# Dahan-Wang/Rethinking-Flow-and-Diffusion-Bridge-Models-for-Speech-Enhancement

Hardware: NVIDIA B200
Metric: enhanced audio-sec/sec (5-step SB bridge, ncsnpp_v2) (higher is better)
Workload: dtype fp16

## Files before the change

rethinking-flow-and-diffusion-bridge-models-for-speech-enhancement_b200/csrc/conv_igemm.cu:

```cuda
#include <cuda.h>
#include <mutex>
#include <type_traits>
#include "common.cuh"
#include "tc05.cuh"

namespace fdbm {
int make_act_tile_map(CUtensorMap* map, const op_t* ptr, int B, int T, int F, int C, int box_f, int box_t);
namespace {

using namespace tc05;

constexpr int MT = 2;
constexpr int TILE_T = 16, TILE_F = 8;
constexpr int HALO_T = TILE_T + 2, HALO_F = TILE_F + 2;
constexpr int A_TILE_BYTES = HALO_T * HALO_F * 128;
constexpr int A_TILE_STRIDE = 23552;
#ifndef FDBM_A_STAGES
#define FDBM_A_STAGES 3
#define FDBM_B_STAGES 3
#endif
constexpr int A_STAGES = FDBM_A_STAGES;
constexpr int B_STAGES = FDBM_B_STAGES;
constexpr int BN = 128;
constexpr int B_TILE_BYTES = BN * 128;
// ... 506 lines not shown
              const float* pb = p.pyr_prev + static_cast<int64_t>(tc.b) * Tp * Fp * p.pyr_C;
              if (p.pyr_C == 4) {
                float4 tap[4];
                float wg[4];
#pragma unroll
                for (int u = 0; u < 2; ++u)
#pragma unroll
                  for (int w = 0; w < 2; ++w) {
                    const int tt = t_a + u, ff = f_a + w;
                    const bool ok = tt >= 0 && tt < Tp && ff >= 0 && ff < Fp;
                    wg[u * 2 + w] = ok ? (u ? 1.0f - wt_a : wt_a) * (w ? 1.0f - wf_a : wf_a) : 0.f;
                    tap[u * 2 + w] = ok ? __ldg(reinterpret_cast<const float4*>(pb + (static_cast<int64_t>(tt) * Fp + ff) * 4))
                                        : make_float4(0.f, 0.f, 0.f, 0.f);
                  }
#pragma unroll
                for (int k = 0; k < 4; ++k) {
                  o[0] = fmaf(wg[k], tap[k].x, o[0]); o[1] = fmaf(wg[k], tap[k].y, o[1]);
                  o[2] = fmaf(wg[k], tap[k].z, o[2]); o[3] = fmaf(wg[k], tap[k].w, o[3]);
                }
              } else {
#pragma unroll
                for (int u = 0; u < 2; ++u) {
                  const int tt = t_a + u;
                  if (tt < 0 || tt >= Tp) continue;
                  const float wt = u ? 1.0f - wt_a : wt_a;
#pragma unroll
                  for (int w = 0; w < 2; ++w) {
                    const int ff = f_a + w;
                    if (ff < 0 || ff >= Fp) continue;
                    const float wgt = wt * (w ? 1.0f - wf_a : wf_a);
                    const float* src = pb + (static_cast<int64_t>(tt) * Fp + ff) * p.pyr_C;
                    for (int c = 0; c < p.pyr_C; ++c) o[c] = fmaf(wgt, __ldg(src + c), o[c]);
                  }
                }
              }
            }
            float* dst = p.pyr_out + ((static_cast<int64_t>(tc.b) * p.T + t) * p.F + f) * p.pyr_C;
            if (p.pyr_C == 4) *reinterpret_cast<float4*>(dst) = make_float4(o[0], o[1], o[2], o[3]);
            else for (int c = 0; c < p.pyr_C; ++c) dst[c] = o[c];
          }
          continue;
        }
        const bool full = tc.t0 + TILE_T <= p.T && tc.f0 + TILE_F <= p.F;
        const int64_t tile_base = ((static_cast<int64_t>(tc.b) * p.T + tc.t0) * p.F + tc.f0) * p.Cout + n0 + cc * 4;
        const int roff0 = ((q * 4) * p.F + rsub) * p.Cout, roff_t = p.F * p.Cout, roff_f = 4 * p.Cout;
        auto roff = [&](int it) { return roff0 + (it >> 1) * roff_t + (it & 1) * roff_f; };
        uint32_t okmask = 0;
#pragma unroll
        for (int it = 0; it < 8; ++it) {
          const int m = q * 32 + it * 4 + rsub;
          const bool ok = tc.t0 + (m >> 3) < p.T && tc.f0 + (m & 7) < p.F;
          okmask |= ok ? (1u << it) : 0u;
        }
        const float* res_p = !RES16 && p.residual ? p.residual + tile_base : nullptr;
        const op_t* res16_p = RES16 ? p.residual_h16 + tile_base : nullptr;
        float* of_p = p.out_f32 ? p.out_f32 + tile_base : nullptr;
        op_t* oh_p = p.out_h16 ? p.out_h16 + tile_base : nullptr;
        if (RES16 || res_p) {
          const int nitem = item + gridDim.x;
          const int nct = item_tile(p, nitem);
          const int nmi = nitem < p.n_items ? nct * MT + j : p.n_mtiles;
          const int nblk_n = nitem - nct * p.n_nblocks;
          const TileCoord nt = decode_tile(p, nmi);
          const int t = nt.t0 + (et >> 3), f = nt.f0 + (et & 7);
          if (nt.valid && t < p.T && f < p.F) {
            const int64_t po = ((static_cast<int64_t>(nt.b) * p.T + t) * p.F + f) * p.Cout + nblk_n * BN;
            if (RES16) {
#pragma unroll
              for (int u = 0; u < 2; ++u) asm volatile("prefetch.global.L2 [%0];" ::"l"(p.residual_h16 + po + u * 64));
            } else {
#pragma unroll
              for (int u = 0; u < 4; ++u) asm volatile("prefetch.global.L2 [%0];" ::"l"(p.residual + po + u * 32));
            }
          }
        }
        const float2 sc2 = make_float2(p.scale, p.scale);
        const float* bias_p = p.bias + n0 + cc * 4;
        const float* biasb_p = p.bias_b ? p.bias_b + static_cast<int64_t>(tc.b) * p.bias_b_stride + n0 + cc * 4 : nullptr;
        float4 bv = __ldg(reinterpret_cast<const float4*>(bias_p));
        float4 bvb = biasb_p ? __ldg(reinterpret_cast<const float4*>(biasb_p)) : make_float4(0.f, 0.f, 0.f, 0.f);
        float4 res[8];
#if FDBM_EPI_RES2
        uint2 res16_buf[2][8];
#define res16 res16_buf[ch & 1]
        auto load_res16 = [&](int ch) {
          uint2 (&dst)[8] = res16_buf[ch & 1];
          if (full) {
#pragma unroll
            for (int it = 0; it < 8; ++it) dst[it] = __ldg(reinterpret_cast<const uint2*>(res16_p + roff(it) + ch * 32));
          } else {
#pragma unroll
            for (int it = 0; it < 8; ++it)
              dst[it] = ((okmask >> it) & 1) ? __ldg(reinterpret_cast<const uint2*>(res16_p + roff(it) + ch * 32)) : make_uint2(0u, 0u);
          }
        };
        if (RES16) load_res16(0);
#else
        uint2 res16[8];
        auto load_res16 = [&](int ch) {
          if (full) {
#pragma unroll
            for (int it = 0; it < 8; ++it) res16[it] = __ldg(reinterpret_cast<const uint2*>(res16_p + roff(it) + ch * 32));
          } else {
#pragma unroll
            for (int it = 0; it < 8; ++it)
              res16[it] = ((okmask >> it) & 1) ? __ldg(reinterpret_cast<const uint2*>(res16_p + roff(it) + ch * 32)) : make_uint2(0u, 0u);
          }
        };
#endif
        auto load_res = [&](float4 (&r)[8], int ch) {
          if (full) {
#pragma unroll
            for (int it = 0; it < 8; ++it) r[it] = __ldg(reinterpret_cast<const float4*>(res_p + roff(it) + ch * 32));
          } else {
#pragma unroll
            for (int it = 0; it < 8; ++it)
              r[it] = ((okmask >> it) & 1) ? __ldg(reinterpret_cast<const float4*>(res_p + roff(it) + ch * 32))
                                           : make_float4(0.f, 0.f, 0.f, 0.f);
          }
        };
        const int n_chunks = p.bn >> 5;
#pragma unroll
        for (int ch = 0; ch < BN / 32; ++ch) {
          if (ch >= n_chunks) break;
          float4 cw[4], cbias = make_float4(0.f, 0.f, 0.f, 0.f);
          if constexpr (COMB) {
            const int c = n0 + ch * 32 + cc * 4;
            cbias = __ldg(reinterpret_cast<const float4*>(p.comb_b + c));
#pragma unroll
            for (int u = 0; u < 4; ++u) {
              const float* wr = p.comb_w + (c + u) * p.comb_C;
              cw[u] = make_float4(__ldg(wr), p.comb_C > 1 ? __ldg(wr + 1) : 0.f, p.comb_C > 2 ? __ldg(wr + 2) : 0.f,
                                  p.comb_C > 3 ? __ldg(wr + 3) : 0.f);
            }
          }
          float4 bvn = bv, bvbn = bvb;
          if (ch + 1 < n_chunks) {
            bvn = __ldg(reinterpret_cast<const float4*>(bias_p + (ch + 1) * 32));
            if (biasb_p) bvbn = __ldg(reinterpret_cast<const float4*>(biasb_p + (ch + 1) * 32));
          }
          uint32_t v[32];
          tmem_ld_32x32(tmem_base + ((q * 32u) << 16) + (as * MT + j) * BN + ch * 32, v);
#if FDBM_EPI_RES2
          if (RES16) { if (ch + 1 < n_chunks) load_res16(ch + 1); }
          else if (res_p) load_res(res, ch);
#else
          if (RES16) { if (ch == 0) load_res16(0); }
          else if (res_p) load_res(res, ch);
#endif
          tmem_ld_wait();
#pragma unroll
          for (int g = 0; g < 8; ++g)
            stage[lane * 8 + (g ^ (lane & 7))] = make_float4(__uint_as_float(v[4 * g]), __uint_as_float(v[4 * g + 1]),
                                                             __uint_as_float(v[4 * g + 2]), __uint_as_float(v[4 * g + 3]));
          __syncwarp();
          const float2 bs_lo = __fmul2_rn(make_float2(bv.x + bvb.x, bv.y + bvb.y), sc2), bs_hi = __fmul2_rn(make_float2(bv.z + bvb.z, bv.w + bvb.w), sc2);
          float2 o_lo[8], o_hi[8];
#pragma unroll
          for (int it = 0; it < 8; ++it) {
            const int rr = it * 4 + rsub;
            const float4 a = stage[rr * 8 + (cc ^ (rr & 7))];
            o_lo[it] = make_float2(a.x, a.y); o_hi[it] = make_float2(a.z, a.w);
          }
#pragma unroll
          for (int it = 0; it < 8; ++it) {
            o_lo[it] = __ffma2_rn(o_lo[it], sc2, bs_lo); o_hi[it] = __ffma2_rn(o_hi[it], sc2, bs_hi);
            if (RES16) {
              const op2_t* r2 = reinterpret_cast<const op2_t*>(&res16[it]);
              o_lo[it] = __ffma2_rn(op22f2(r2[0]), sc2, o_lo[it]);
              o_hi[it] = __ffma2_rn(op22f2(r2[1]), sc2, o_hi[it]);
            } else if (res_p) {
              o_lo[it] = __ffma2_rn(make_float2(res[it].x, res[it].y), sc2, o_lo[it]);
              o_hi[it] = __ffma2_rn(make_float2(res[it].z, res[it].w), sc2, o_hi[it]);
            }
            if (COMB && (full || ((okmask >> it) & 1))) {
              const int m = q * 32 + it * 4 + rsub;
              const float* pq = p.comb_pyr + ((static_cast<int64_t>(tc.b) * p.T + tc.t0 + (m >> 3)) * p.F + tc.f0 + (m & 7)) * p.comb_C;
              const float p0 = __ldg(pq), p1 = p.comb_C > 1 ? __ldg(pq + 1) : 0.f, p2 = p.comb_C > 2 ? __ldg(pq + 2) : 0.f,
                          p3 = p.comb_C > 3 ? __ldg(pq + 3) : 0.f;
              o_lo[it].x += cbias.x + cw[0].x * p0 + cw[0].y * p1 + cw[0].z * p2 + cw[0].w * p3;
              o_lo[it].y += cbias.y + cw[1].x * p0 + cw[1].y * p1 + cw[1].z * p2 + cw[1].w * p3;
              o_hi[it].x += cbias.z + cw[2].x * p0 + cw[2].y * p1 + cw[2].z * p2 + cw[2].w * p3;
              o_hi[it].y += cbias.w + cw[3].x * p0 + cw[3].y * p1 + cw[3].z * p2 + cw[3].w * p3;
            }
          }
#if !FDBM_EPI_RES2
          if (RES16 && ch + 1 < n_chunks) load_res16(ch + 1);
#endif
          float2 ssum_lo = make_float2(0.f, 0.f), ssum_hi = ssum_lo, ssq_lo = ssum_lo, ssq_hi = ssum_lo;
          if (full) {
            if (of_p) {
#pragma unroll
              for (int it = 0; it < 8; ++it)
                *reinterpret_cast<float4*>(of_p + roff(it) + ch * 32) = make_float4(o_lo[it].x, o_lo[it].y, o_hi[it].x, o_hi[it].y);
            }
            if (oh_p) {
#pragma unroll
              for (int it = 0; it < 8; ++it)
                *reinterpret_cast<uint2*>(oh_p + roff(it) + ch * 32) = make_uint2(pack_op2(o_lo[it].x, o_lo[it].y), pack_op2(o_hi[it].x, o_hi[it].y));
            }
#pragma unroll
            for (int it = 0; it < 8; ++it) {
              ssum_lo = __fadd2_rn(ssum_lo, o_lo[it]); ssum_hi = __fadd2_rn(ssum_hi, o_hi[it]);
              ssq_lo = __ffma2_rn(o_lo[it], o_lo[it], ssq_lo); ssq_hi = __ffma2_rn(o_hi[it], o_hi[it], ssq_hi);
            }
          } else {
#pragma unroll
            for (int it = 0; it < 8; ++it) {
              if ((okmask >> it) & 1) {
                if (of_p) *reinterpret_cast<float4*>(of_p + roff(it) + ch * 32) = make_float4(o_lo[it].x, o_lo[it].y, o_hi[it].x, o_hi[it].y);
                if (oh_p) *reinterpret_cast<uint2*>(oh_p + roff(it) + ch * 32) = make_uint2(pack_op2(o_lo[it].x, o_lo[it].y), pack_op2(o_hi[it].x, o_hi[it].y));
                ssum_lo = __fadd2_rn(ssum_lo, o_lo[it]); ssum_hi = __fadd2_rn(ssum_hi, o_hi[it]);
                ssq_lo = __ffma2_rn(o_lo[it], o_lo[it], ssq_lo); ssq_hi = __ffma2_rn(o_hi[it], o_hi[it], ssq_hi);
              }
            }
          }
          float4 ssum = make_float4(ssum_lo.x, ssum_lo.y, ssum_hi.x, ssum_hi.y), ssq = make_float4(ssq_lo.x, ssq_lo.y, ssq_hi.x, ssq_hi.y);
          if (do_stats) {
#pragma unroll
            for (int sft = 8; sft <= 16; sft <<= 1) {
              ssum.x += __shfl_xor_sync(0xffffffffu, ssum.x, sft); ssum.y += __shfl_xor_sync(0xffffffffu, ssum.y, sft);
              ssum.z += __shfl_xor_sync(0xffffffffu, ssum.z, sft); ssum.w += __shfl_xor_sync(0xffffffffu, ssum.w, sft);
              ssq.x += __shfl_xor_sync(0xffffffffu, ssq.x, sft); ssq.y += __shfl_xor_sync(0xffffffffu, ssq.y, sft);
              ssq.z += __shfl_xor_sync(0xffffffffu, ssq.z, sft); ssq.w += __shfl_xor_sync(0xffffffffu, ssq.w, sft);
            }
            if (rsub == 0) {
              float4* d = reinterpret_cast<float4*>(wstat + q * BN + ch * 32 + cc * 4);
              d[0] = make_float4(ssum.x, ssq.x, ssum.y, ssq.y);
              d[1] = make_float4(ssum.z, ssq.z, ssum.w, ssq.w);
            }
          }
          __syncwarp();
// ... 153 lines not shown
  PackDesc d{};
  d.w1 = w; d.w2 = nullptr; d.out = wpack; d.kind = 1; d.C1 = Cin; d.ksize = k; d.io = ksize == -1; d.C2 = Cin_total ? Cin_total : Cin; d.Cout = Cout;
  d.rows_total = 0; d.row_offset = ci_off;
  d.total = static_cast<long long>(Cout / 64) * k * k * Cin * 64;
  return d;
}
int launch_pack_batch(const PackDesc* descs_dev, int n_descs, long long n_blocks, cudaStream_t s) {
  if (n_descs <= 0 || n_blocks <= 0) return FDBM_OK;
  pack_batch_kernel<<<static_cast<unsigned>(n_blocks), 256, 0, s>>>(descs_dev, n_descs);
  FDBM_LAUNCH_CHECK();
  return FDBM_OK;
}

__global__ void __launch_bounds__(256) pack_one_kernel(const PackDesc d) {
  for (int64_t i = blockIdx.x * 256ll + threadIdx.x; i < d.total; i += 256ll * gridDim.x) {
    if (d.kind == 0) pack_fwd_element(d, i); else pack_dgrad_element(d, i);
  }
}

int launch_pack_conv_weights(const float* w1, int C1, int ksize, const float* w2, int C2, int Cout, int n_rows_total,
                             int row_offset, op_t* wpack, cudaStream_t s) {
  FDBM_REQUIRE((ksize == -2 && C1 <= 4 && C2 == 0) ||
               (C1 % 64 == 0 && C2 % 64 == 0 && (ksize == 1 || ksize == 3 || ksize == -1)),
               "pack_conv_weights: channels must be multiples of 64, ksize 1 or 3");
  const PackDesc d = pack_desc_fwd(w1, C1, ksize, w2, C2, Cout, n_rows_total, row_offset, wpack);
  pack_one_kernel<<<static_cast<int>(std::min<int64_t>(ceil_div64(d.total, 256), 4096)), 256, 0, s>>>(d);
  FDBM_LAUNCH_CHECK();
  return FDBM_OK;
}

int launch_pack_conv_weights_dgrad(const float* w, int Cout, int Cin, int ksize, op_t* wpack, cudaStream_t s, int Cin_total, int ci_off) {
  FDBM_REQUIRE(Cout % 64 == 0 && Cin % 64 == 0 && (ksize == 1 || ksize == 3 || ksize == -1),
               "pack_conv_weights_dgrad: channels must be multiples of 64, ksize 1, 3 or -1 (NIN)");
  const PackDesc d = pack_desc_dgrad(w, Cout, Cin, ksize, wpack, Cin_total, ci_off);
  pack_one_kernel<<<static_cast<int>(std::min<int64_t>(ceil_div64(d.total, 256), 4096)), 256, 0, s>>>(d);
  FDBM_LAUNCH_CHECK();
  return FDBM_OK;
}

int launch_conv_igemm(const ConvArgs& a, cudaStream_t s) {
  FDBM_REQUIRE(a.n_seg >= 1 && a.n_seg <= MAX_SEG, "conv_igemm: 1..%d K segments", MAX_SEG);
  const int bn = a.narrow_n ? 16 : (a.Cout == 64 ? 64 : BN);
  FDBM_REQUIRE(a.Cout % bn == 0 && (!a.narrow_n || (a.Cout == 16 && a.pyr_out)), "conv_igemm: Cout must be a multiple of %d (got %d)", bn, a.Cout);
  FDBM_REQUIRE(a.out_f32 || a.out_h16 || a.pyr_out, "conv_igemm: no output");
  FDBM_REQUIRE(!a.pyr_out || (a.pyr_C >= 1 && a.pyr_C <= 4 && a.Cout == bn && !a.sums), "conv_igemm: bad pyramid epilogue arguments");
  FDBM_REQUIRE(!a.pyr_prev || (a.T % 2 == 0 && a.F % 2 == 0), "conv_igemm: pyramid level with odd size");
  static PerDeviceOnce attr_once;
  if (attr_once.first(current_device())) {
    FDBM_CUDA(cudaFuncSetAttribute(conv_igemm_kernel<false, false>, cudaFuncAttributeMaxDynamicSharedMemorySize, SMEM_BYTES));
    FDBM_CUDA(cudaFuncSetAttribute(conv_igemm_kernel<false, true>, cudaFuncAttributeMaxDynamicSharedMemorySize, SMEM_BYTES));
    FDBM_CUDA(cudaFuncSetAttribute(conv_igemm_kernel<true, false>, cudaFuncAttributeMaxDynamicSharedMemorySize, SMEM_BYTES));
  }
  FDBM_REQUIRE(!a.comb_pyr || (a.comb_w && a.comb_b && a.comb_C >= 1 && a.comb_C <= 4 && !a.pyr_out), "conv_igemm: bad Combine epilogue arguments");
  CUtensorMap map_a[MAX_SEG], map_b;
  ConvParams p;
  p.B = a.B; p.T = a.T; p.F = a.F; p.Cout = a.Cout;
  p.n_seg = a.n_seg;
  int kb = 0, n_kt = 0;
  for (int i = 0; i < MAX_SEG; ++i) {
    if (i < a.n_seg) {
      const ConvSeg& sg = a.seg[i];
      FDBM_REQUIRE(sg.in && sg.C > 0 && sg.C % 64 == 0 && (sg.taps == 9 || sg.taps == 1),
                   "conv_igemm: segment %d needs a tensor, C %% 64 == 0 and 9 or 1 taps (C=%d, taps=%d)", i, sg.C, sg.taps);
      const int halo = sg.taps == 9 || sg.norm_tab != nullptr;
      if (int rc = halo ? make_act_map(&map_a[i], sg.in, a.B, a.T, a.F, sg.C)
                        : make_act_tile_map(&map_a[i], sg.in, a.B, a.T, a.F, sg.C, TILE_F, TILE_T)) return rc;
      p.seg[i].halo = halo;
      kb += sg.C / 64; p.seg[i].taps = sg.taps;
      p.seg[i].norm = sg.norm_tab != nullptr; p.seg[i].act = sg.act; p.seg[i].tab = sg.norm_tab;
      p.seg[i].tab_stride = sg.tab_stride;
      n_kt += (sg.C / 64) * sg.taps;
    } else {
      map_a[i] = map_a[0];
      p.seg[i] = SegParams{1, 0, 0, 0, 0, nullptr};
    }
  }
  p.n_kb = kb;
  FDBM_REQUIRE(kb <= MAX_KB, "conv_igemm: at most %d K-blocks (got %d)", MAX_KB, kb);
  {
    uint32_t nine[MAX_KB], one[MAX_KB];
    int n9 = 0, n1 = 0, kt = 0;
    for (int i = 0; i < a.n_seg; ++i)
      for (int cb = 0; cb < a.seg[i].C / 64; ++cb) {
        const uint32_t e = static_cast<uint32_t>(i) | (static_cast<uint32_t>(cb) << 4) | (static_cast<uint32_t>(kt) << 16);
        if (a.seg[i].taps == 9) nine[n9++] = e; else one[n1++] = e;
        kt += a.seg[i].taps;
      }
    static const int order = getenv("FDBM_KSCHED") ? atoi(getenv("FDBM_KSCHED")) : 0;
    int n = 0;
    if (order == 1) {
      for (int i = 0; i < n1; ++i) p.ksched[n++] = one[i];
      for (int i = 0; i < n9; ++i) p.ksched[n++] = nine[i];
    } else if (order == 2 && n9 > 0) {
      p.ksched[n++] = nine[0];
      for (int i = 0; i < n1; ++i) p.ksched[n++] = one[i];
      for (int i = 1; i < n9; ++i) p.ksched[n++] = nine[i];
    } else {
      for (int i = 0; i < n9; ++i) p.ksched[n++] = nine[i];
      for (int i = 0; i < n1; ++i) p.ksched[n++] = one[i];
    }
    for (; n < MAX_KB; ++n) p.ksched[n] = 0;
    bool side_ok = order == 0 && n1 > 0 && n9 > 0;
    for (int i = 0; i < a.n_seg; ++i) side_ok = side_ok && (a.seg[i].taps == 9 || !p.seg[i].halo);
    static const int side_env = getenv("FDBM_SIDE_RING") ? atoi(getenv("FDBM_SIDE_RING")) : FDBM_SIDE_RING_DEFAULT;
    p.side_ring = side_ok && side_env ? 1 : 0;
    p.n_main = p.side_ring ? n9 : kb;
    p.side_gap = p.side_ring ? std::max(3, ceil_div(9 * n9, n1)) : 0;
    p.n_steps = n_kt;
  }
  if (int rc = make_weight_map(&map_b, a.wpack, static_cast<int64_t>(n_kt) * a.Cout, bn)) return rc;
  p.bn = bn;
  p.tiles_t = ceil_div(a.T, TILE_T); p.tiles_f = ceil_div(a.F, TILE_F);
  p.n_mtiles = a.B * p.tiles_t * p.tiles_f;
  p.n_nblocks = a.Cout / bn;
  p.n_items = ceil_div(p.n_mtiles, MT) * p.n_nblocks;
  {
    auto magic = [](int d) { return static_cast<uint32_t>((0x100000000ull + d - 1) / static_cast<uint64_t>(d)); };
    p.mg_tiles_t = magic(p.tiles_t); p.mg_tiles_f = magic(p.tiles_f); p.mg_nblocks = magic(p.n_nblocks);
    const int64_t dmax = std::max(std::max(p.tiles_t, p.tiles_f), p.n_nblocks);
    FDBM_REQUIRE((2 * (static_cast<int64_t>(p.n_items) + num_sms()) + 2) * dmax < 0x100000000ll, "conv_igemm: %d items exceed the range of the index arithmetic", p.n_items);
  }
  p.bias = a.bias; p.bias_b = a.bias_b; p.bias_b_stride = a.bias_b_stride; p.residual = a.residual; p.scale = a.scale;
  p.residual_h16 = a.residual_h16;
  FDBM_REQUIRE(!(a.residual && a.residual_h16) && !(a.residual_h16 && (a.comb_pyr || a.pyr_out)), "conv_igemm: bad residual arguments");
  p.out_f32 = a.out_f32; p.out_h16 = a.out_h16; p.sums = a.sums;
  p.pyr_out = a.pyr_out; p.pyr_prev = a.pyr_prev; p.pyr_C = a.pyr_C;
  p.comb_pyr = a.comb_pyr; p.comb_w = a.comb_w; p.comb_b = a.comb_b; p.comb_C = a.comb_C;
  if (a.sums) {
    FDBM_REQUIRE(p.n_nblocks <= STAT_SLOTS, "conv_igemm: channel sums support Cout <= %d", STAT_SLOTS * BN);
    if (!a.sums_prezeroed) FDBM_CUDA(cudaMemsetAsync(a.sums, 0, sizeof(double) * 2 * a.B * a.Cout, s));
  }
  const int grid = std::min(p.n_items, num_sms());
  cudaLaunchConfig_t cfg = {};
  cfg.gridDim = dim3(grid); cfg.blockDim = dim3(NUM_THREADS); cfg.dynamicSmemBytes = SMEM_BYTES; cfg.stream = s;
  cudaLaunchAttribute attr[1];
  attr[0].id = cudaLaunchAttributeProgrammaticStreamSerialization;
  attr[0].val.programmaticStreamSerializationAllowed = 1;
  cfg.attrs = attr; cfg.numAttrs = pdl_enabled() && a.B <= pdl_batch_limit() ? 1 : 0;
  if (a.comb_pyr) FDBM_CUDA(cudaLaunchKernelEx(&cfg, conv_igemm_kernel<true, false>, map_a[0], map_a[1], map_a[2], map_b, p));
  else if (a.residual_h16) FDBM_CUDA(cudaLaunchKernelEx(&cfg, conv_igemm_kernel<false, true>, map_a[0], map_a[1], map_a[2], map_b, p));
  else FDBM_CUDA(cudaLaunchKernelEx(&cfg, conv_igemm_kernel<false, false>, map_a[0], map_a[1], map_a[2], map_b, p));
  FDBM_LAUNCH_CHECK();
  return FDBM_OK;
}

}

using namespace fdbm;

extern "C" int fdbm_pack_conv_weights(const float* w1, int C1, int ksize, const float* w2, int C2, int Cout,
                                      void* wpack, int64_t* bytes, void* stream) {
  const int k = ksize == -1 ? 1 : ksize;
  if (bytes) *bytes = ksize == -2 ? static_cast<int64_t>(Cout) * 64 * 2 : conv_wpack_bytes(C1, k, C2, Cout);
  if (!wpack) return FDBM_OK;
  if (int rc = require_sm100()) return rc;
  FDBM_REQUIRE(w1 && ((C2 == 0) == (w2 == nullptr)), "fdbm_pack_conv_weights: null pointer");
  FDBM_REQUIRE(ksize != -2 || (C1 >= 1 && 9 * C1 <= 64 && C2 == 0), "fdbm_pack_conv_weights: ksize -2 needs 9 * C1 <= 64 and no second operand");
  return launch_pack_conv_weights(w1, C1, ksize, w2, C2, Cout, Cout, 0, reinterpret_cast<op_t*>(wpack),
                                  as_stream(stream));
}

extern "C" int fdbm_pack_conv_weights_dgrad(const float* w, int Cout, int Cin, int ksize, void* wpack, int64_t* bytes,
                                            void* stream) {
  const int k = ksize == -1 ? 1 : ksize;
  if (bytes) *bytes = conv_wpack_bytes(Cout, k, 0, Cin);
  if (!wpack) return FDBM_OK;
  if (int rc = require_sm100()) return rc;
  FDBM_REQUIRE(w, "fdbm_pack_conv_weights_dgrad: null weights");
  return launch_pack_conv_weights_dgrad(w, Cout, Cin, ksize, reinterpret_cast<op_t*>(wpack), as_stream(stream));
}

extern "C" int fdbm_conv_igemm(const void* in1, int C1, int ksize, const void* in2, int C2, const void* wpack,
                               const float* bias, const float* bias_b, const float* residual, float scale, int batch,
                               int T, int F, int Cout, float* out_f32, void* out_h16, double* sums, void* stream) {
  if (int rc = require_sm100()) return rc;
  FDBM_REQUIRE(in1 && wpack && bias && batch > 0 && T > 0 && F > 0, "fdbm_conv_igemm: bad arguments");
  FDBM_REQUIRE(ksize == 1 || ksize == 3, "fdbm_conv_igemm: ksize must be 1 or 3");
// ... 34 lines not shown
```

rethinking-flow-and-diffusion-bridge-models-for-speech-enhancement_b200/csrc/norm_resample.cu:

```cuda
#include "common.cuh"

namespace fdbm {
namespace {

struct Taps1D {
  int n;
  int pos[4];
  float w[4];
};

__device__ __forceinline__ Taps1D taps_for(int o, int mode) {
  Taps1D t;
  if (mode == 1) {
    t.n = 4;
    t.pos[0] = 2 * o - 1; t.pos[1] = 2 * o; t.pos[2] = 2 * o + 1; t.pos[3] = 2 * o + 2;
    t.w[0] = 0.125f; t.w[1] = 0.375f; t.w[2] = 0.375f; t.w[3] = 0.125f;
  } else if (mode == 2) {
    const int i = o >> 1;
    t.n = 2;
    if (o & 1) { t.pos[0] = i; t.pos[1] = i + 1; t.w[0] = 0.75f; t.w[1] = 0.25f; }
    else       { t.pos[0] = i - 1; t.pos[1] = i; t.w[0] = 0.25f; t.w[1] = 0.75f; }
    t.pos[2] = t.pos[3] = -1; t.w[2] = t.w[3] = 0.f;
  } else {
    t.n = 1; t.pos[0] = o; t.w[0] = 1.f;
    t.pos[1] = t.pos[2] = t.pos[3] = -1; t.w[1] = t.w[2] = t.w[3] = 0.f;
  }
  return t;
}

__host__ __device__ inline int out_dim(int n, int mode) { return mode == 1 ? n / 2 : (mode == 2 ? n * 2 : n); }

__global__ void __launch_bounds__(256)
fir_resample_kernel(const float* __restrict__ in, int B, int T, int F, int C, int mode, float scale, float* __restrict__ out) {
  const int To = out_dim(T, mode), Fo = out_dim(F, mode);
  const int64_t total = static_cast<int64_t>(B) * To * Fo * C;
  for (int64_t i = blockIdx.x * 256ll + threadIdx.x; i < total; i += 256ll * gridDim.x) {
    const int c = static_cast<int>(i % C);
    int64_t p = i / C;
    const int fo = static_cast<int>(p % Fo); p /= Fo;
    const int to = static_cast<int>(p % To);
    const int b = static_cast<int>(p / To);
    const Taps1D tt = taps_for(to, mode), tf = taps_for(fo, mode);
    float acc = 0.f;
    for (int a = 0; a < tt.n; ++a) {
      if (tt.pos[a] < 0 || tt.pos[a] >= T) continue;
      for (int q = 0; q < tf.n; ++q) {
        if (tf.pos[q] < 0 || tf.pos[q] >= F) continue;
        acc += tt.w[a] * tf.w[q] * in[((static_cast<int64_t>(b) * T + tt.pos[a]) * F + tf.pos[q]) * C + c];
      }
    }
    out[i] = acc * scale;
  }
}

__global__ void __launch_bounds__(256)
channel_stats_kernel(const float* __restrict__ in, int64_t P, int C, int64_t px_per_block, double* __restrict__ sums) {
  __shared__ float4 red_s[256], red_q[256];
  const int cg = C / 4;
  const int pl = 256 / cg;
  const int ci = threadIdx.x % cg, pi = threadIdx.x / cg;
  const int b = blockIdx.y;
  const int64_t p0 = blockIdx.x * px_per_block;
  const int64_t p1 = min(P, p0 + px_per_block);
  float4 s = make_float4(0.f, 0.f, 0.f, 0.f), q = s;
  if (pi < pl) {
    const float4* base = reinterpret_cast<const float4*>(in + static_cast<int64_t>(b) * P * C) + ci;
    for (int64_t p = p0 + pi; p < p1; p += pl) {
      const float4 v = base[p * cg];
      s.x += v.x; s.y += v.y; s.z += v.z; s.w += v.w;
      q.x += v.x * v.x; q.y += v.y * v.y; q.z += v.z * v.z; q.w += v.w * v.w;
    }
  }
  red_s[threadIdx.x] = s;
  red_q[threadIdx.x] = q;
  __syncthreads();
  if (threadIdx.x < cg) {
    double ds[4] = {0, 0, 0, 0}, dq[4] = {0, 0, 0, 0};
    for (int j = 0; j < pl; ++j) {
      const float4 a = red_s[j * cg + threadIdx.x], c2 = red_q[j * cg + threadIdx.x];
      ds[0] += a.x; ds[1] += a.y; ds[2] += a.z; ds[3] += a.w;
      dq[0] += c2.x; dq[1] += c2.y; dq[2] += c2.z; dq[3] += c2.w;
    }
    double* o = sums + (static_cast<int64_t>(b) * C + threadIdx.x * 4) * 2;
#pragma unroll
    for (int j = 0; j < 4; ++j) {
      atomicAdd(o + 2 * j, ds[j]);
      atomicAdd(o + 2 * j + 1, dq[j]);
    }
  }
}

constexpr int GN_MAXC = 512;


template <int MODE, bool SRC16>
__global__ void __launch_bounds__(256)
groupnorm_act_kernel(const void* __restrict__ src1, const double* __restrict__ sums1, int C1,
                     const void* __restrict__ src2, const double* __restrict__ sums2, int C2,
                     const float* __restrict__ gamma, const float* __restrict__ beta, int T, int F, int silu,
                     int px_per_block, uint4* __restrict__ act_out, uint4* __restrict__ raw_out) {
  pdl_wait_then_trigger();
  __shared__ float sA[GN_MAXC], sB[GN_MAXC];
  __shared__ float s_mean[32], s_rstd[32];
  const int C = C1 + C2;
  const int b = blockIdx.y;
// ... 41 lines not shown

  const int To = out_dim(T, MODE), Fo = out_dim(F, MODE);
  const int n_px = To * Fo;
  const int p0 = blockIdx.x * px_per_block;
  const int p1 = min(n_px, p0 + px_per_block);
  constexpr int NT = MODE == 1 ? 4 : (MODE == 2 ? 2 : 1);
  for (int p = p0 + pl; p < p1; p += npl) {
    const int fo = p % Fo, to = p / Fo;
    float acc[8], raw[8];
#pragma unroll
    for (int j = 0; j < 8; ++j) { acc[j] = 0.f; raw[j] = 0.f; }
    const Taps1D tt = taps_for(to, MODE), tf = taps_for(fo, MODE);
#pragma unroll
    for (int u = 0; u < NT; ++u) {
      if (tt.pos[u] < 0 || tt.pos[u] >= T) continue;
#pragma unroll
      for (int v = 0; v < NT; ++v) {
        if (tf.pos[v] < 0 || tf.pos[v] >= F) continue;
        const float w = tt.w[u] * tf.w[v];
        const int64_t off = (static_cast<int64_t>(tt.pos[u]) * F + tf.pos[v]) * Cs + cs;
        float x[8];
        if (SRC16) {
          const uint4 rawv = *reinterpret_cast<const uint4*>(sh + off);
          const op2_t* h2 = reinterpret_cast<const op2_t*>(&rawv);
#pragma unroll
          for (int j = 0; j < 4; ++j) { const float2 f2 = op22f2(h2[j]); x[2 * j] = f2.x; x[2 * j + 1] = f2.y; }
        } else {
          const float4 x0 = *reinterpret_cast<const float4*>(sf + off), x1 = *reinterpret_cast<const float4*>(sf + off + 4);
          x[0] = x0.x; x[1] = x0.y; x[2] = x0.z; x[3] = x0.w; x[4] = x1.x; x[5] = x1.y; x[6] = x1.z; x[7] = x1.w;
        }
#pragma unroll
        for (int j = 0; j < 8; ++j) {
          float y = fmaf(x[j], a[j], bb[j]);
          if (silu) {
            float th;
            asm("tanh.approx.f32 %0, %1;" : "=f"(th) : "f"(0.5f * y));
            y *= fmaf(th, 0.5f, 0.5f);
          }
          acc[j] = fmaf(w, y, acc[j]);
          raw[j] = fmaf(w, x[j], raw[j]);
        }
      }
    }
    const int64_t o = (static_cast<int64_t>(b) * n_px + p) * cg8 + g8;
    act_out[o] = make_uint4(pack_op2(acc[0], acc[1]), pack_op2(acc[2], acc[3]), pack_op2(acc[4], acc[5]),
                            pack_op2(acc[6], acc[7]));
    if (raw_out)
      raw_out[o] = make_uint4(pack_op2(raw[0], raw[1]), pack_op2(raw[2], raw[3]), pack_op2(raw[4], raw[5]),
                              pack_op2(raw[6], raw[7]));
  }
}

constexpr int RS_ROWS = 16;

template <int MODE>
__global__ void __launch_bounds__(256, 2)
gn_resample16_kernel(const op_t* __restrict__ src1, int C1, const op_t* __restrict__ src2, int C2,
                     const float2* __restrict__ tab, int B, int T, int F, op_t* __restrict__ act_out,
                     op_t* __restrict__ raw_out) {
  const int C = C1 + C2, C4 = C / 4;
  const int To = MODE == 1 ? T / 2 : T * 2, Fo = MODE == 1 ? F / 2 : F * 2;
  const int nstrip = MODE == 1 ? (Fo + 1) / 2 : (F + 1) / 2;
  const int nrows = MODE == 1 ? To : T;
  const int nchunk = (nrows + RS_ROWS - 1) / RS_ROWS;
  int64_t idx = blockIdx.x * 256ll + threadIdx.x;
  if (idx >= static_cast<int64_t>(B) * nchunk * nstrip * C4) return;
  const int cg = static_cast<int>(idx % C4); idx /= C4;
  const int strip = static_cast<int>(idx % nstrip); idx /= nstrip;
  const int chunk = static_cast<int>(idx % nchunk);
  const int b = static_cast<int>(idx / nchunk);
  const int c0 = cg * 4;
  const bool from2 = c0 >= C1;
  const int Cs = from2 ? C2 : C1;
  const op_t* sp = (from2 ? src2 : src1) + static_cast<int64_t>(b) * T * F * Cs + (from2 ? c0 - C1 : c0);
  float2 sc[2], sh[2];
  {
    const float4* tp = reinterpret_cast<const float4*>(tab + static_cast<int64_t>(b) * C + c0);
    const float4 e0 = __ldg(tp), e1 = __ldg(tp + 1);
    sc[0] = make_float2(0.5f * e0.x, 0.5f * e0.z); sh[0] = make_float2(0.5f * e0.y, 0.5f * e0.w);
    sc[1] = make_float2(0.5f * e1.x, 0.5f * e1.z); sh[1] = make_float2(0.5f * e1.y, 0.5f * e1.w);
  }
  auto px_act = [&](const uint2 rawv, float2 (&a)[2], float2 (&r)[2]) {
    const op2_t* h2 = reinterpret_cast<const op2_t*>(&rawv);
#pragma unroll
    for (int w = 0; w < 2; ++w) {
      r[w] = op22f2(h2[w]);
      const float2 y = __ffma2_rn(r[w], sc[w], sh[w]);
      const op2_t h = f2op2(y.x, y.y);
      a[w] = op22f2(__hfma2(h, op2_tanh(h), h));
    }
  };
  auto store_px = [&](int to, int fo, const float2 (&a)[2], const float2 (&r)[2]) {
    if (fo >= Fo) return;
    const int64_t o = ((static_cast<int64_t>(b) * To + to) * Fo + fo) * C + c0;
    *reinterpret_cast<uint2*>(act_out + o) = make_uint2(pack_op2(a[0].x, a[0].y), pack_op2(a[1].x, a[1].y));
    *reinterpret_cast<uint2*>(raw_out + o) = make_uint2(pack_op2(r[0].x, r[0].y), pack_op2(r[1].x, r[1].y));
  };
  const float2 zero2 = make_float2(0.f, 0.f);

  if (MODE == 1) {
    const int fo0 = 2 * strip, fi0 = 2 * fo0 - 1;
    uint32_t okf = 0;
#pragma unroll
    for (int k = 0; k < 6; ++k) okf |= (fi0 + k >= 0 && fi0 + k < F) ? (1u << k) : 0u;
    const float2 w1 = make_float2(0.125f, 0.125f), w3 = make_float2(0.375f, 0.375f);
    auto load_row = [&](int t, uint2 (&raw)[6]) {
      const bool in = t >= 0 && t < T;
      const op_t* rp = sp + (static_cast<int64_t>(in ? t : 0) * F + fi0) * Cs;
#pragma unroll
      for (int k = 0; k < 6; ++k) raw[k] = (in && ((okf >> k) & 1)) ? __ldg(reinterpret_cast<const uint2*>(rp + k * Cs)) : make_uint2(0u, 0u);
    };
    auto hrow = [&](int t, const uint2 (&raw)[6], float2 (&ha)[2][2], float2 (&hr)[2][2]) {
#pragma unroll
      for (int j = 0; j < 2; ++j) { ha[j][0] = zero2; ha[j][1] = zero2; hr[j][0] = zero2; hr[j][1] = zero2; }
      if (t < 0 || t >= T) return;
#pragma unroll
      for (int k = 0; k < 6; ++k) {
        float2 a[2], r[2];
        px_act(raw[k], a, r);
        if (!((okf >> k) & 1)) { a[0] = zero2; a[1] = zero2; }
        if (k < 4) {
          const float2 w = (k == 0 || k == 3) ? w1 : w3;
#pragma unroll
          for (int c = 0; c < 2; ++c) { ha[0][c] = __ffma2_rn(w, a[c], ha[0][c]); hr[0][c] = __ffma2_rn(w, r[c], hr[0][c]); }
        }
        if (k >= 2) {
          const float2 w = (k == 2 || k == 5) ? w1 : w3;
#pragma unroll
          for (int c = 0; c < 2; ++c) { ha[1][c] = __ffma2_rn(w, a[c], ha[1][c]); hr[1][c] = __ffma2_rn(w, r[c], hr[1][c]); }
        }
      }
    };
    const int to0 = chunk * RS_ROWS, to1 = min(To, to0 + RS_ROWS);
    float2 ca[2][2], cr[2][2], na[2][2], nr[2][2], ha[2][2], hr[2][2];
    uint2 ra[6], rb[6], qa[6], qb[6];
    load_row(2 * to0 - 1, ra); load_row(2 * to0, rb);
    load_row(2 * to0 + 1, qa); load_row(2 * to0 + 2, qb);
    hrow(2 * to0 - 1, ra, ha, hr);
#pragma unroll
    for (int j = 0; j < 2; ++j)
#pragma unroll
      for (int c = 0; c < 2; ++c) { ca[j][c] = __fmul2_rn(w1, ha[j][c]); cr[j][c] = __fmul2_rn(w1, hr[j][c]); }
    hrow(2 * to0, rb, ha, hr);
#pragma unroll
    for (int j = 0; j < 2; ++j)
#pragma unroll
      for (int c = 0; c < 2; ++c) { ca[j][c] = __ffma2_rn(w3, ha[j][c], ca[j][c]); cr[j][c] = __ffma2_rn(w3, hr[j][c], cr[j][c]); }
#pragma unroll 1
    for (int to = to0; to < to1; ++to) {
#pragma unroll
      for (int k = 0; k < 6; ++k) { ra[k] = qa[k]; rb[k] = qb[k]; }
      if (to + 1 < to1) { load_row(2 * to + 3, qa); load_row(2 * to + 4, qb); }
      hrow(2 * to + 1, ra, ha, hr);
#pragma unroll
      for (int j = 0; j < 2; ++j)
#pragma unroll
        for (int c = 0; c < 2; ++c) {
          ca[j][c] = __ffma2_rn(w3, ha[j][c], ca[j][c]); cr[j][c] = __ffma2_rn(w3, hr[j][c], cr[j][c]);
          na[j][c] = __fmul2_rn(w1, ha[j][c]); nr[j][c] = __fmul2_rn(w1, hr[j][c]);
        }
      hrow(2 * to + 2, rb, ha, hr);
#pragma unroll
      for (int j = 0; j < 2; ++j) {
#pragma unroll
        for (int c = 0; c < 2; ++c) {
          ca[j][c] = __ffma2_rn(w1, ha[j][c], ca[j][c]); cr[j][c] = __ffma2_rn(w1, hr[j][c], cr[j][c]);
          na[j][c] = __ffma2_rn(w3, ha[j][c], na[j][c]); nr[j][c] = __ffma2_rn(w3, hr[j][c], nr[j][c]);
        }
        store_px(to, fo0 + j, ca[j], cr[j]);
#pragma unroll
        for (int c = 0; c < 2; ++c) { ca[j][c] = na[j][c]; cr[j][c] = nr[j][c]; }
      }
    }
  } else {
    const int f0 = 2 * strip;
    uint32_t okf = 0;
#pragma unroll
    for (int k = 0; k < 4; ++k) okf |= (f0 - 1 + k >= 0 && f0 - 1 + k < F) ? (1u << k) : 0u;
    const float2 q1 = make_float2(0.25f, 0.25f), q3 = make_float2(0.75f, 0.75f);
    auto hrow = [&](int t, float2 (&ha)[4][2], float2 (&hr)[4][2]) {
      float2 a[4][2], r[4][2];
      if (t < 0 || t >= T) {
#pragma unroll
        for (int k = 0; k < 4; ++k) { ha[k][0] = zero2; ha[k][1] = zero2; hr[k][0] = zero2; hr[k][1] = zero2; }
        return;
      }
      const op_t* rp = sp + (static_cast<int64_t>(t) * F + f0 - 1) * Cs;
      uint2 raw[4];
#pragma unroll
      for (int k = 0; k < 4; ++k) raw[k] = ((okf >> k) & 1) ? __ldg(reinterpret_cast<const uint2*>(rp + k * Cs)) : make_uint2(0u, 0u);
#pragma unroll
      for (int k = 0; k < 4; ++k) {
        px_act(raw[k], a[k], r[k]);
        if (!((okf >> k) & 1)) { a[k][0] = zero2; a[k][1] = zero2; }
      }
#pragma unroll
      for (int c = 0; c < 2; ++c) {
        ha[0][c] = __ffma2_rn(q1, a[0][c], __fmul2_rn(q3, a[1][c])); hr[0][c] = __ffma2_rn(q1, r[0][c], __fmul2_rn(q3, r[1][c]));
        ha[1][c] = __ffma2_rn(q3, a[1][c], __fmul2_rn(q1, a[2][c])); hr[1][c] = __ffma2_rn(q3, r[1][c], __fmul2_rn(q1, r[2][c]));
        ha[2][c] = __ffma2_rn(q1, a[1][c], __fmul2_rn(q3, a[2][c])); hr[2][c] = __ffma2_rn(q1, r[1][c], __fmul2_rn(q3, r[2][c]));
        ha[3][c] = __ffma2_rn(q3, a[2][c], __fmul2_rn(q1, a[3][c])); hr[3][c] = __ffma2_rn(q3, r[2][c], __fmul2_rn(q1, r[3][c]));
      }
    };
    const int i0 = chunk * RS_ROWS, i1 = min(T, i0 + RS_ROWS);
    float2 pa[4][2], pr[4][2], qa[4][2], qr[4][2];
    hrow(i0 - 1, pa, pr);
#pragma unroll 1
    for (int i = i0; i <= i1; ++i) {
      hrow(i, qa, qr);
#pragma unroll
      for (int k = 0; k < 4; ++k) {
        float2 oa[2], orr[2];
        if (i > i0) {
#pragma unroll
// ... 44 lines not shown
    }
    const double cnt = cpg * pixels;
    const double mean = s / cnt;
    double var = q / cnt - mean * mean;
    if (var < 0) var = 0;
    s_mean[threadIdx.x] = static_cast<float>(mean);
    s_rstd[threadIdx.x] = static_cast<float>(1.0 / sqrt(var + 1e-6));
    if (stats) stats[static_cast<int64_t>(b) * G + threadIdx.x] = make_float2(s_mean[threadIdx.x], s_rstd[threadIdx.x]);
  }
  __syncthreads();
#pragma unroll
  for (int u = 0; u < GN_MAXC / 256; ++u) {
    const int c = threadIdx.x + u * 256;
    if (c < C) {
      if (blk_real && (c & 127) >= blk_real) { table[static_cast<int64_t>(b) * C + c] = make_float2(0.f, 0.f); continue; }
      const int g = (blk_real ? (c >> 7) * blk_real + (c & 127) : c) / cpg;
      const float a = gam[u] * s_rstd[g];
      table[static_cast<int64_t>(b) * C + c] = make_float2(a, bet[u] - s_mean[g] * a);
    }
  }
}

}

int launch_gn_finalize(const double* sums1, int C1, const double* sums2, int C2, const float* gamma, const float* beta,
                       int B, int64_t pixels, float2* table, cudaStream_t s, int blk_real, float2* stats) {
  const int C = C1 + C2;
  FDBM_REQUIRE(blk_real == 0 || (blk_real > 0 && blk_real < 128 && blk_real % 4 == 0 && C1 % 128 == 0 && C2 % 128 == 0),
               "gn_finalize: channel_block_real %d needs 128-channel blocks (%d+%d)", blk_real, C1, C2);
  const int Cr = blk_real ? C / 128 * blk_real : C;
  FDBM_REQUIRE(Cr % std::min(Cr / 4, 32) == 0 && C >= 4 && C <= GN_MAXC, "gn_finalize: unsupported channels %d+%d", C1, C2);
  cudaLaunchConfig_t cfg = {};
  cfg.gridDim = dim3(B); cfg.blockDim = dim3(256); cfg.stream = s;
  cudaLaunchAttribute attr[1];
  attr[0].id = cudaLaunchAttributeProgrammaticStreamSerialization;
  attr[0].val.programmaticStreamSerializationAllowed = 1;
  cfg.attrs = attr; cfg.numAttrs = pdl_enabled() && B <= pdl_batch_limit() ? 1 : 0;
  FDBM_CUDA(cudaLaunchKernelEx(&cfg, gn_finalize_kernel, sums1, C1, sums2, C2, gamma, beta, static_cast<double>(pixels), table, blk_real, stats));
  FDBM_LAUNCH_CHECK();
  return FDBM_OK;
}

int launch_gn_resample16(const op_t* src1, int C1, const op_t* src2, int C2, const float2* tab, int B, int T, int F,
                         int mode, op_t* act_out, op_t* raw_out, cudaStream_t s) {
  const int C = C1 + C2;
  FDBM_REQUIRE(src1 && tab && act_out && raw_out && C1 % 4 == 0 && C2 % 4 == 0 && (C2 == 0) == (src2 == nullptr),
               "gn_resample16: bad arguments (channels %d+%d)", C1, C2);
  FDBM_REQUIRE(mode == 1 || mode == 2, "gn_resample16: mode must be 1 (down) or 2 (up)");
  FDBM_REQUIRE(mode != 1 || (T % 2 == 0 && F % 2 == 0), "gn_resample16: down-sampling needs even T, F");
  const int nstrip = mode == 1 ? (F / 2 + 1) / 2 : (F + 1) / 2;
  const int nrows = mode == 1 ? T / 2 : T;
  const int64_t total = static_cast<int64_t>(B) * ceil_div(nrows, RS_ROWS) * nstrip * (C / 4);
  const unsigned grid = static_cast<unsigned>(ceil_div64(total, 256));
  if (mode == 1) gn_resample16_kernel<1><<<grid, 256, 0, s>>>(src1, C1, src2, C2, tab, B, T, F, act_out, raw_out);
  else gn_resample16_kernel<2><<<grid, 256, 0, s>>>(src1, C1, src2, C2, tab, B, T, F, act_out, raw_out);
  FDBM_LAUNCH_CHECK();
  return FDBM_OK;
}

int launch_fir_resample(const float* in, int B, int T, int F, int C, int mode, float* out, cudaStream_t s) {
  return launch_fir_resample_scaled(in, B, T, F, C, mode, 1.0f, out, s);
}

int launch_fir_resample_scaled(const float* in, int B, int T, int F, int C, int mode, float scale, float* out, cudaStream_t s) {
  const int64_t total = static_cast<int64_t>(B) * out_dim(T, mode) * out_dim(F, mode) * C;
  const int grid = static_cast<int>(std::min<int64_t>(ceil_div64(total, 256), static_cast<int64_t>(num_sms()) * 16));
  fir_resample_kernel<<<grid, 256, 0, s>>>(in, B, T, F, C, mode, scale, out);
  FDBM_LAUNCH_CHECK();
  return FDBM_OK;
}

int launch_channel_stats(const float* in, int B, int T, int F, int C, double* sums, cudaStream_t s) {
  FDBM_REQUIRE(C % 4 == 0 && C / 4 <= 256 && 256 % (C / 4) == 0, "channel_stats: unsupported channel count %d", C);
  FDBM_CUDA(cudaMemsetAsync(sums, 0, sizeof(double) * 2 * B * C, s));
  const int64_t P = static_cast<int64_t>(T) * F;
  const int pl = 256 / (C / 4);
  int64_t blocks_x = std::max<int64_t>(1, (static_cast<int64_t>(num_sms()) * 8) / B);
  blocks_x = std::min<int64_t>(blocks_x, std::max<int64_t>(1, P / (pl * 8)));
  const int64_t ppb = ceil_div64(P, blocks_x);
  dim3 grid(static_cast<unsigned>(ceil_div64(P, ppb)), B);
  channel_stats_kernel<<<grid, 256, 0, s>>>(in, P, C, ppb, sums);
  FDBM_LAUNCH_CHECK();
  return FDBM_OK;
}

int launch_groupnorm_act(const void* src1, int src1_h16, const double* sums1, int C1, const void* src2,
                         const double* sums2, int C2, const float* gamma, const float* beta, int B, int T, int F,
                         int silu, int mode, op_t* act_out, op_t* raw_out, cudaStream_t s) {
  const int C = C1 + C2;
  FDBM_REQUIRE(C <= GN_MAXC && C1 % 8 == 0 && C2 % 8 == 0 && C % std::min(C / 4, 32) == 0 && C / 8 <= 256,
               "groupnorm_act: unsupported channels %d+%d", C1, C2);
  FDBM_REQUIRE(mode >= 0 && mode <= 2, "groupnorm_act: bad mode %d", mode);
  FDBM_REQUIRE(mode != 1 || (T % 2 == 0 && F % 2 == 0), "groupnorm_act: down-sampling needs even T, F");
  const int n_px = out_dim(T, mode) * out_dim(F, mode);
  const int npl = 256 / (C / 8);
  int blocks_x = std::max(1, (num_sms() * 8) / B);
  blocks_x = std::min(blocks_x, std::max(1, n_px / (npl * 4)));
  const int ppb = ceil_div(ceil_div(n_px, blocks_x), npl) * npl;
  dim3 grid(ceil_div(n_px, ppb), B);
  uint4* ao = reinterpret_cast<uint4*>(act_out);
  uint4* ro = reinterpret_cast<uint4*>(raw_out);
#define FDBM_GN_LAUNCH(M, H) \
  FDBM_CUDA(launch_maybe_pdl(groupnorm_act_kernel<M, H>, grid, dim3(256), 0, s, pdl_enabled() && B <= pdl_batch_limit(), src1, sums1, C1, src2, sums2, C2, \
                             gamma, beta, T, F, silu, ppb, ao, ro))
  if (src1_h16) {
    if (mode == 0) FDBM_GN_LAUNCH(0, true); else if (mode == 1) FDBM_GN_LAUNCH(1, true); else FDBM_GN_LAUNCH(2, true);
  } else {
    if (mode == 0) FDBM_GN_LAUNCH(0, false); else if (mode == 1) FDBM_GN_LAUNCH(1, false); else FDBM_GN_LAUNCH(2, false);
  }
#undef FDBM_GN_LAUNCH
  FDBM_LAUNCH_CHECK();
  return FDBM_OK;
}

}

using namespace fdbm;

// ... 38 lines not shown
```

Measured before the change: 1354.

## Hoist Combine pyramid loads, vectorize FIR resample, cp.async ring in down-resample

The Combine epilogue now loads each pixel's pyramid values once per tile, as float4 when four channels are present, instead of reloading them per channel chunk. It also prefetches the next tile's pyramid data and reads the combine weights as float4. A float4 FIR resample kernel replaces the scalar one when alignment and sizes allow. The down-sampling GN resample kernel now streams input rows through a multi-stage cp.async shared-memory ring instead of register double-buffering, which costs dynamic shared memory and could reduce occupancy.

```diff
diff --git a/rethinking-flow-and-diffusion-bridge-models-for-speech-enhancement_b200/csrc/conv_igemm.cu b/rethinking-flow-and-diffusion-bridge-models-for-speech-enhancement_b200/csrc/conv_igemm.cu
--- a/rethinking-flow-and-diffusion-bridge-models-for-speech-enhancement_b200/csrc/conv_igemm.cu
+++ b/rethinking-flow-and-diffusion-bridge-models-for-speech-enhancement_b200/csrc/conv_igemm.cu
@@ -582,7 +582,7 @@
           const bool ok = tc.t0 + (m >> 3) < p.T && tc.f0 + (m & 7) < p.F;
           okmask |= ok ? (1u << it) : 0u;
         }
-        const float* res_p = !RES16 && p.residual ? p.residual + tile_base : nullptr;
+        const float* res_p = !RES16 && !COMB && p.residual ? p.residual + tile_base : nullptr;
         const op_t* res16_p = RES16 ? p.residual_h16 + tile_base : nullptr;
         float* of_p = p.out_f32 ? p.out_f32 + tile_base : nullptr;
         op_t* oh_p = p.out_h16 ? p.out_h16 + tile_base : nullptr;
@@ -649,6 +649,23 @@
                                            : make_float4(0.f, 0.f, 0.f, 0.f);
           }
         };
+        float4 pyr[8];
+        if constexpr (COMB) {
+          const float* pq = p.comb_pyr + ((static_cast<int64_t>(tc.b) * p.T + tc.t0) * p.F + tc.f0) * p.comb_C;
+#pragma unroll
+          for (int it = 0; it < 8; ++it) {
+            const int m = q * 32 + it * 4 + rsub;
+            const float* px = pq + ((m >> 3) * p.F + (m & 7)) * p.comb_C;
+            if (!full && !((okmask >> it) & 1)) pyr[it] = make_float4(0.f, 0.f, 0.f, 0.f);
+            else if (p.comb_C == 4) pyr[it] = __ldg(reinterpret_cast<const float4*>(px));
+            else pyr[it] = make_float4(__ldg(px), p.comb_C > 1 ? __ldg(px + 1) : 0.f, p.comb_C > 2 ? __ldg(px + 2) : 0.f, 0.f);
+          }
+          const int nitem = item + gridDim.x;
+          const TileCoord nt = decode_tile(p, nitem < p.n_items ? item_tile(p, nitem) * MT + j : p.n_mtiles);
+          const int t = nt.t0 + (et >> 3), f = nt.f0 + (et & 7);
+          if (nt.valid && t < p.T && f < p.F)
+            asm volatile("prefetch.global.L2 [%0];" ::"l"(p.comb_pyr + ((static_cast<int64_t>(nt.b) * p.T + t) * p.F + f) * p.comb_C));
+        }
         const int n_chunks = p.bn >> 5;
 #pragma unroll
         for (int ch = 0; ch < BN / 32; ++ch) {
@@ -660,8 +677,8 @@
 #pragma unroll
             for (int u = 0; u < 4; ++u) {
               const float* wr = p.comb_w + (c + u) * p.comb_C;
-              cw[u] = make_float4(__ldg(wr), p.comb_C > 1 ? __ldg(wr + 1) : 0.f, p.comb_C > 2 ? __ldg(wr + 2) : 0.f,
-                                  p.comb_C > 3 ? __ldg(wr + 3) : 0.f);
+              cw[u] = p.comb_C == 4 ? __ldg(reinterpret_cast<const float4*>(wr))
+                                    : make_float4(__ldg(wr), p.comb_C > 1 ? __ldg(wr + 1) : 0.f, p.comb_C > 2 ? __ldg(wr + 2) : 0.f, 0.f);
             }
           }
           float4 bvn = bv, bvbn = bvb;
@@ -704,10 +721,7 @@
               o_hi[it] = __ffma2_rn(make_float2(res[it].z, res[it].w), sc2, o_hi[it]);
             }
             if (COMB && (full || ((okmask >> it) & 1))) {
-              const int m = q * 32 + it * 4 + rsub;
-              const float* pq = p.comb_pyr + ((static_cast<int64_t>(tc.b) * p.T + tc.t0 + (m >> 3)) * p.F + tc.f0 + (m & 7)) * p.comb_C;
-              const float p0 = __ldg(pq), p1 = p.comb_C > 1 ? __ldg(pq + 1) : 0.f, p2 = p.comb_C > 2 ? __ldg(pq + 2) : 0.f,
-                          p3 = p.comb_C > 3 ? __ldg(pq + 3) : 0.f;
+              const float p0 = pyr[it].x, p1 = pyr[it].y, p2 = pyr[it].z, p3 = pyr[it].w;
               o_lo[it].x += cbias.x + cw[0].x * p0 + cw[0].y * p1 + cw[0].z * p2 + cw[0].w * p3;
               o_lo[it].y += cbias.y + cw[1].x * p0 + cw[1].y * p1 + cw[1].z * p2 + cw[1].w * p3;
               o_hi[it].x += cbias.z + cw[2].x * p0 + cw[2].y * p1 + cw[2].z * p2 + cw[2].w * p3;
@@ -967,6 +981,8 @@
     FDBM_CUDA(cudaFuncSetAttribute(conv_igemm_kernel<true, false>, cudaFuncAttributeMaxDynamicSharedMemorySize, SMEM_BYTES));
   }
   FDBM_REQUIRE(!a.comb_pyr || (a.comb_w && a.comb_b && a.comb_C >= 1 && a.comb_C <= 4 && !a.pyr_out), "conv_igemm: bad Combine epilogue arguments");
+  FDBM_REQUIRE(!a.comb_pyr || a.comb_C != 4 || ((reinterpret_cast<uintptr_t>(a.comb_pyr) | reinterpret_cast<uintptr_t>(a.comb_w)) & 15) == 0,
+               "conv_igemm: the 4-channel Combine pyramid and weights must be 16-byte aligned");
   CUtensorMap map_a[MAX_SEG], map_b;
   ConvParams p;
   p.B = a.B; p.T = a.T; p.F = a.F; p.Cout = a.Cout;
@@ -1037,7 +1053,7 @@
   }
   p.bias = a.bias; p.bias_b = a.bias_b; p.bias_b_stride = a.bias_b_stride; p.residual = a.residual; p.scale = a.scale;
   p.residual_h16 = a.residual_h16;
-  FDBM_REQUIRE(!(a.residual && a.residual_h16) && !(a.residual_h16 && (a.comb_pyr || a.pyr_out)), "conv_igemm: bad residual arguments");
+  FDBM_REQUIRE(!(a.residual && a.residual_h16) && !((a.residual || a.residual_h16) && (a.comb_pyr || a.pyr_out)), "conv_igemm: bad residual arguments");
   p.out_f32 = a.out_f32; p.out_h16 = a.out_h16; p.sums = a.sums;
   p.pyr_out = a.pyr_out; p.pyr_prev = a.pyr_prev; p.pyr_C = a.pyr_C;
   p.comb_pyr = a.comb_pyr; p.comb_w = a.comb_w; p.comb_b = a.comb_b; p.comb_C = a.comb_C;
diff --git a/rethinking-flow-and-diffusion-bridge-models-for-speech-enhancement_b200/csrc/norm_resample.cu b/rethinking-flow-and-diffusion-bridge-models-for-speech-enhancement_b200/csrc/norm_resample.cu
--- a/rethinking-flow-and-diffusion-bridge-models-for-speech-enhancement_b200/csrc/norm_resample.cu
+++ b/rethinking-flow-and-diffusion-bridge-models-for-speech-enhancement_b200/csrc/norm_resample.cu
@@ -51,6 +51,31 @@
     }
     out[i] = acc * scale;
   }
+}
+
+__global__ void __launch_bounds__(256)
+fir_resample4_kernel(const float4* __restrict__ in, int T, int F, int C4, int mode, float scale, float4* __restrict__ out) {
+  const int To = out_dim(T, mode), Fo = out_dim(F, mode);
+  const int i = blockIdx.x * 256 + threadIdx.x;
+  if (i >= To * Fo * C4) return;
+  const int b = blockIdx.y;
+  const int c = i % C4, px = i / C4;
+  const int fo = px % Fo, to = px / Fo;
+  const float4* src = in + static_cast<int64_t>(b) * T * F * C4 + c;
+  const Taps1D tt = taps_for(to, mode), tf = taps_for(fo, mode);
+  float4 acc = make_float4(0.f, 0.f, 0.f, 0.f);
+#pragma unroll
+  for (int a = 0; a < 4; ++a) {
+    if (a >= tt.n || tt.pos[a] < 0 || tt.pos[a] >= T) continue;
+#pragma unroll
+    for (int q = 0; q < 4; ++q) {
+      if (q >= tf.n || tf.pos[q] < 0 || tf.pos[q] >= F) continue;
+      const float w = tt.w[a] * tf.w[q];
+      const float4 x = __ldg(src + (tt.pos[a] * F + tf.pos[q]) * C4);
+      acc.x += w * x.x; acc.y += w * x.y; acc.z += w * x.z; acc.w += w * x.w;
+    }
+  }
+  out[static_cast<int64_t>(b) * To * Fo * C4 + i] = make_float4(acc.x * scale, acc.y * scale, acc.z * scale, acc.w * scale);
 }
 
 __global__ void __launch_bounds__(256)
@@ -198,12 +223,25 @@
 }
 
 constexpr int RS_ROWS = 16;
+#ifndef FDBM_RS_STAGES
+#define FDBM_RS_STAGES 3
+#endif
+constexpr int RS_STAGES = FDBM_RS_STAGES;
+constexpr int RS_RING_BYTES = RS_STAGES * 12 * 256 * 8;
+
+__device__ __forceinline__ void cp_async8(void* dst, const void* src, bool ok) {
+  asm volatile("cp.async.ca.shared.global [%0], [%1], 8, %2;" ::"r"(static_cast<uint32_t>(__cvta_generic_to_shared(dst))), "l"(src), "r"(ok ? 8 : 0) : "memory");
+}
+__device__ __forceinline__ void cp_async_commit() { asm volatile("cp.async.commit_group;" ::: "memory"); }
+template <int N>
+__device__ __forceinline__ void cp_async_wait() { asm volatile("cp.async.wait_group %0;" ::"n"(N) : "memory"); }
 
 template <int MODE>
 __global__ void __launch_bounds__(256, 2)
 gn_resample16_kernel(const op_t* __restrict__ src1, int C1, const op_t* __restrict__ src2, int C2,
                      const float2* __restrict__ tab, int B, int T, int F, op_t* __restrict__ act_out,
                      op_t* __restrict__ raw_out) {
+  extern __shared__ uint2 rs_ring[];
   const int C = C1 + C2, C4 = C / 4;
   const int To = MODE == 1 ? T / 2 : T * 2, Fo = MODE == 1 ? F / 2 : F * 2;
   const int nstrip = MODE == 1 ? (Fo + 1) / 2 : (F + 1) / 2;
@@ -250,11 +288,32 @@
 #pragma unroll
     for (int k = 0; k < 6; ++k) okf |= (fi0 + k >= 0 && fi0 + k < F) ? (1u << k) : 0u;
     const float2 w1 = make_float2(0.125f, 0.125f), w3 = make_float2(0.375f, 0.375f);
-    auto load_row = [&](int t, uint2 (&raw)[6]) {
-      const bool in = t >= 0 && t < T;
-      const op_t* rp = sp + (static_cast<int64_t>(in ? t : 0) * F + fi0) * Cs;
-#pragma unroll
-      for (int k = 0; k < 6; ++k) raw[k] = (in && ((okf >> k) & 1)) ? __ldg(reinterpret_cast<const uint2*>(rp + k * Cs)) : make_uint2(0u, 0u);
+    const int to0 = chunk * RS_ROWS, to1 = min(To, to0 + RS_ROWS);
+    uint2* ring = rs_ring + threadIdx.x;
+    const int npair = to1 - to0 + 1;
+    const int pt0 = 2 * to0 - 1;
+    auto issue_pair = [&](int k) {
+      if (k < npair) {
+        uint2* dst = ring + (k % RS_STAGES) * 12 * 256;
+#pragma unroll
+        for (int r = 0; r < 2; ++r) {
+          const int t = pt0 + 2 * k + r;
+          const bool in = t >= 0 && t < T;
+          const op_t* rp = sp + (static_cast<int64_t>(in ? t : 0) * F + fi0) * Cs;
+#pragma unroll
+          for (int kk = 0; kk < 6; ++kk) {
+            const bool ok = in && ((okf >> kk) & 1);
+            cp_async8(dst + (r * 6 + kk) * 256, ok ? rp + kk * Cs : sp, ok);
+          }
+        }
+      }
+      cp_async_commit();
+    };
+    auto read_pair = [&](int k, uint2 (&ra)[6], uint2 (&rb)[6]) {
+      cp_async_wait<RS_STAGES - 1>();
+      const uint2* src = ring + (k % RS_STAGES) * 12 * 256;
+#pragma unroll
+      for (int kk = 0; kk < 6; ++kk) { ra[kk] = src[kk * 256]; rb[kk] = src[(6 + kk) * 256]; }
     };
     auto hrow = [&](int t, const uint2 (&raw)[6], float2 (&ha)[2][2], float2 (&hr)[2][2]) {
 #pragma unroll
@@ -277,11 +336,11 @@
         }
       }
     };
-    const int to0 = chunk * RS_ROWS, to1 = min(To, to0 + RS_ROWS);
     float2 ca[2][2], cr[2][2], na[2][2], nr[2][2], ha[2][2], hr[2][2];
-    uint2 ra[6], rb[6], qa[6], qb[6];
-    load_row(2 * to0 - 1, ra); load_row(2 * to0, rb);
-    load_row(2 * to0 + 1, qa); load_row(2 * to0 + 2, qb);
+    uint2 ra[6], rb[6];
+#pragma unroll
+    for (int k = 0; k < RS_STAGES; ++k) issue_pair(k);
+    read_pair(0, ra, rb);
     hrow(2 * to0 - 1, ra, ha, hr);
 #pragma unroll
     for (int j = 0; j < 2; ++j)
@@ -292,11 +351,11 @@
     for (int j = 0; j < 2; ++j)
 #pragma unroll
       for (int c = 0; c < 2; ++c) { ca[j][c] = __ffma2_rn(w3, ha[j][c], ca[j][c]); cr[j][c] = __ffma2_rn(w3, hr[j][c], cr[j][c]); }
+    issue_pair(RS_STAGES);
 #pragma unroll 1
     for (int to = to0; to < to1; ++to) {
-#pragma unroll
-      for (int k = 0; k < 6; ++k) { ra[k] = qa[k]; rb[k] = qb[k]; }
-      if (to + 1 < to1) { load_row(2 * to + 3, qa); load_row(2 * to + 4, qb); }
+      const int k = to - to0 + 1;
+      read_pair(k, ra, rb);
       hrow(2 * to + 1, ra, ha, hr);
 #pragma unroll
       for (int j = 0; j < 2; ++j)
@@ -306,6 +365,7 @@
           na[j][c] = __fmul2_rn(w1, ha[j][c]); nr[j][c] = __fmul2_rn(w1, hr[j][c]);
         }
       hrow(2 * to + 2, rb, ha, hr);
+      issue_pair(k + RS_STAGES);
 #pragma unroll
       for (int j = 0; j < 2; ++j) {
 #pragma unroll
@@ -456,7 +516,10 @@
   const int nrows = mode == 1 ? T / 2 : T;
   const int64_t total = static_cast<int64_t>(B) * ceil_div(nrows, RS_ROWS) * nstrip * (C / 4);
   const unsigned grid = static_cast<unsigned>(ceil_div64(total, 256));
-  if (mode == 1) gn_resample16_kernel<1><<<grid, 256, 0, s>>>(src1, C1, src2, C2, tab, B, T, F, act_out, raw_out);
+  static PerDeviceOnce attr_once;
+  if (attr_once.first(current_device()))
+    FDBM_CUDA(cudaFuncSetAttribute(gn_resample16_kernel<1>, cudaFuncAttributeMaxDynamicSharedMemorySize, RS_RING_BYTES));
+  if (mode == 1) gn_resample16_kernel<1><<<grid, 256, RS_RING_BYTES, s>>>(src1, C1, src2, C2, tab, B, T, F, act_out, raw_out);
   else gn_resample16_kernel<2><<<grid, 256, 0, s>>>(src1, C1, src2, C2, tab, B, T, F, act_out, raw_out);
   FDBM_LAUNCH_CHECK();
   return FDBM_OK;
@@ -467,7 +530,15 @@
 }
 
 int launch_fir_resample_scaled(const float* in, int B, int T, int F, int C, int mode, float scale, float* out, cudaStream_t s) {
-  const int64_t total = static_cast<int64_t>(B) * out_dim(T, mode) * out_dim(F, mode) * C;
+  const int64_t per_utt = static_cast<int64_t>(out_dim(T, mode)) * out_dim(F, mode) * C;
+  if (C % 4 == 0 && B <= 65535 && static_cast<int64_t>(T) * F * C < (1ll << 31) && per_utt < (1ll << 31) &&
+      (reinterpret_cast<uintptr_t>(in) & 15) == 0 && (reinterpret_cast<uintptr_t>(out) & 15) == 0) {
+    const dim3 grid(static_cast<unsigned>(ceil_div64(per_utt / 4, 256)), B);
+    fir_resample4_kernel<<<grid, 256, 0, s>>>(reinterpret_cast<const float4*>(in), T, F, C / 4, mode, scale, reinterpret_cast<float4*>(out));
+    FDBM_LAUNCH_CHECK();
+    return FDBM_OK;
+  }
+  const int64_t total = B * per_utt;
   const int grid = static_cast<int>(std::min<int64_t>(ceil_div64(total, 256), static_cast<int64_t>(num_sms()) * 16));
   fir_resample_kernel<<<grid, 256, 0, s>>>(in, B, T, F, C, mode, scale, out);
   FDBM_LAUNCH_CHECK();
```

Measured after the change: 1366 (median of 6 runs). About the same (+0.8%).
